# andyp223/ErasureCodedPIR

Measured on AMD Instinct MI355X. Metric: device-resident shard GiB/s per PIR query, 1/2/4/8 MI355X; bit-exact vs CPU, higher is better.
Workload: dtype u8; 1 GPU; north_star target shape: one shard 2^24 x 1 KiB, DPF depth 24, p=2; records=16777216, record_bytes=1024, parties=2, num_rounds=1, records_per_gpu=16777216, dpf_depth=24, parallelism=single, step=one PIR query: its own DPF key and tree, one full pass over the shard

## Files before the change

### erasurecodedpir_amd/csrc/pir_bits.h

```cpp
#pragma once
#include <stdint.h>

#if defined(__HIPCC__)
#include <hip/hip_runtime.h>
#define PIR_HD __host__ __device__ __forceinline__
#else
#define PIR_HD inline
#endif

namespace pir {

template <int S>
PIR_HD void bit_swap(uint32_t& a, uint32_t& b, uint32_t m) {
  const uint32_t t = ((a >> S) ^ b) & m;
  b ^= t;
  a ^= t << S;
}

PIR_HD void transpose8x32(uint32_t (&x)[8]) {
  bit_swap<4>(x[0], x[4], 0x0F0F0F0Fu); bit_swap<4>(x[1], x[5], 0x0F0F0F0Fu);
  bit_swap<4>(x[2], x[6], 0x0F0F0F0Fu); bit_swap<4>(x[3], x[7], 0x0F0F0F0Fu);
  bit_swap<2>(x[0], x[2], 0x33333333u); bit_swap<2>(x[1], x[3], 0x33333333u);
  bit_swap<2>(x[4], x[6], 0x33333333u); bit_swap<2>(x[5], x[7], 0x33333333u);
  bit_swap<1>(x[0], x[1], 0x55555555u); bit_swap<1>(x[2], x[3], 0x55555555u);
  bit_swap<1>(x[4], x[5], 0x55555555u); bit_swap<1>(x[6], x[7], 0x55555555u);
}

PIR_HD void transpose32(uint32_t (&a)[32]) {
#pragma unroll
  for (int k = 0; k < 16; ++k) bit_swap<16>(a[k], a[k + 16], 0x0000FFFFu);
#pragma unroll
  for (int k = 0; k < 32; ++k)
    if (!(k & 8)) bit_swap<8>(a[k], a[k + 8], 0x00FF00FFu);
#pragma unroll
  for (int k = 0; k < 32; ++k)
    if (!(k & 4)) bit_swap<4>(a[k], a[k + 4], 0x0F0F0F0Fu);
#pragma unroll
  for (int k = 0; k < 32; ++k)
    if (!(k & 2)) bit_swap<2>(a[k], a[k + 2], 0x33333333u);
#pragma unroll
  for (int k = 0; k < 32; ++k)
    if (!(k & 1)) bit_swap<1>(a[k], a[k + 1], 0x55555555u);
}

}
```

### erasurecodedpir_amd/csrc/pir_scan_t.hip

```cpp
#include "pir_bits.h"
#include <stdlib.h>
#include <type_traits>
#include "pir_kernels.h"

namespace pir {

constexpr int kScanTWaves = kScanTThreads / 64;

__device__ __forceinline__ uint32_t gf_xtime4_t(uint32_t x) {
  return ((x & 0x7f7f7f7fu) << 1) ^ (((x >> 7) & 0x01010101u) * 0x1du);
}

template <int NQ, int NRP>
__global__ __launch_bounds__(kScanTThreads) __attribute__((amdgpu_waves_per_eu(kScanTWavesPerEU)))
void k_scan_t(const uint8_t* __restrict__ shard, uint64_t nrec, uint32_t pitch, uint32_t cpr,
              const uint8_t* __restrict__ c, uint8_t* __restrict__ slabs, int accumulate,
              uint32_t ckey, uint64_t ckoff) {
  static_assert(NRP == 4 || NRP == 8, "coefficient words of 32 or 64 bits");
  static_assert(NQ >= 1 && NQ <= NRP, "rounds");
  constexpr int WD = NRP / 4;
  constexpr int GW = kColGroupLanes;
  __shared__ alignas(8) uint32_t tab[kScanTWaves][256 * WD];
  __shared__ uint32_t red[NQ * GW];
  __shared__ uint32_t next_chunk;
  for (int i = threadIdx.x; i < NQ * GW; i += blockDim.x) red[i] = 0;
  const bool dyn = (accumulate >> 1) & 1;
  accumulate &= 1;

  const uint32_t lane = threadIdx.x & 63;
  const uint32_t wv = __builtin_amdgcn_readfirstlane(threadIdx.x >> 6);
  const uint64_t wave = (uint64_t)blockIdx.x * kScanTWaves + wv;
  const uint64_t nwaves = (uint64_t)gridDim.x * kScanTWaves;
  const uint32_t chunk = blockIdx.y * kColGroupLanes + lane;
  const bool active = chunk < cpr;
  const uint64_t r0 = dyn ? (uint64_t)blockIdx.x * kScanTWaves * nrec / nwaves : wave * nrec / nwaves;
  const uint64_t r1 = dyn ? ((uint64_t)blockIdx.x + 1) * kScanTWaves * nrec / nwaves : (wave + 1) * nrec / nwaves;
  uint32_t* const tw = &tab[wv][0];
  if (dyn) {
    if (threadIdx.x == 0) next_chunk = 0;
    __syncthreads();
  }

  uint32_t Zt[32][WD];
#pragma unroll
  for (int j = 0; j < 32; ++j)
#pragma unroll
    for (int d = 0; d < WD; ++d) Zt[j][d] = 0;

  if (r1 > r0) {
    const uint32_t nrows = (uint32_t)(r1 - r0);
    const __amdgpu_buffer_rsrc_t rs = __builtin_amdgcn_make_buffer_rsrc(
        (void*)(shard + r0 * pitch), (short)0, (int)(nrows * pitch), kBufRsrcWord3);
    const uint32_t voff = (active ? chunk : 0u) * 4u;
    auto load_rel = [&](uint32_t rel) __attribute__((always_inline)) {
      return (uint32_t)__builtin_amdgcn_raw_buffer_load_b32(rs, voff, rel < nrows ? rel * pitch : 0u, 2);
    };
    auto coefs64 = [&](uint32_t rb) __attribute__((always_inline)) {
      const uint32_t rl = rb + lane;
      uint2 cw = make_uint2(0, 0);
      if (rl < nrows) {
        const uint64_t row = r0 + rl;
        if (ckey == 0) {
          const uint8_t* p = c + row * NRP;
          if constexpr (NRP == 8) cw = *reinterpret_cast<const uint2*>(p);
          else cw.x = *reinterpret_cast<const uint32_t*>(p);
        } else {
          uint64_t w = 0;
          for (uint32_t g = 0; g * ckey < (uint32_t)NRP; ++g) {
            const uint8_t* p = c + g * ckoff + row * ckey;
            const uint64_t v = ckey == 1 ? *p : (ckey == 2 ? *reinterpret_cast<const uint16_t*>(p)
                                                           : *reinterpret_cast<const uint32_t*>(p));
            w |= v << (8 * g * ckey);
          }
          cw = make_uint2((uint32_t)w, (uint32_t)(w >> 32));
        }
      }
      return cw;
    };
    uint32_t lm[6];
#pragma unroll
    for (int r = 0; r < 6; ++r) lm[r] = ((lane >> r) & 1u) ? 0xffffffffu : 0u;

    const uint32_t nch = (nrows + 63) / 64;
    auto claim = [&]() __attribute__((always_inline)) -> uint32_t {
      uint32_t v = 0;
      if (lane == 0)
        v = __hip_atomic_fetch_add(&next_chunk, 1u, __ATOMIC_RELAXED, __HIP_MEMORY_SCOPE_WORKGROUP);
      return (uint32_t)__builtin_amdgcn_readfirstlane(v);
    };
    uint32_t cur = dyn ? claim() : 0u;
    uint32_t nxt = dyn ? (cur < nch ? claim() : nch) : 1u;
    auto seq_row = [&](uint32_t k) __attribute__((always_inline)) -> uint32_t {
      return k < 64 ? cur * 64 + k : (nxt < nch ? nxt * 64 + (k - 64) : nrows);
    };
    uint32_t x[16];
#pragma unroll
    for (int u = 0; u < 16; ++u) x[u] = load_rel(seq_row((uint32_t)u));
    uint2 cw = cur < nch ? coefs64(cur * 64) : make_uint2(0, 0);
    for (; cur < nch;) {
      const uint32_t rb = cur * 64;
      const uint2 cwn = nxt < nch ? coefs64(nxt * 64) : make_uint2(0, 0);
      const uint32_t nb = nrows - rb < 64 ? nrows - rb : 64;
      for (uint32_t j0 = 0; j0 < nb; j0 += 16) {
#pragma unroll
        for (int g = 0; g < 2; ++g) {
          const uint32_t j = j0 + 8 * g;
#pragma unroll
          for (int d = 0; d < WD; ++d) {
            uint32_t w[8];
#pragma unroll
            for (int r = 0; r < 8; ++r)
              w[r] = (uint32_t)__builtin_amdgcn_readlane((int)(d ? cw.y : cw.x), (int)(j + r));
            uint32_t e = 0;
#pragma unroll
            for (int r = 0; r < 6; ++r) e = __builtin_amdgcn_bitop3_b32(e, w[r], lm[r], 0x78);
            const uint32_t e6 = e ^ w[6], e7 = e ^ w[7];
            tw[lane * WD + d] = e;
            tw[(lane + 64) * WD + d] = e6;
            tw[(lane + 128) * WD + d] = e7;
            tw[(lane + 192) * WD + d] = e6 ^ w[7];
          }
          __builtin_amdgcn_wave_barrier();
          uint32_t (&R)[8] = *reinterpret_cast<uint32_t(*)[8]>(&x[8 * g]);
          transpose8x32(R);
          uint32_t id[32];
#pragma unroll
          for (int jj = 0; jj < 32; ++jj) id[jj] = (R[jj & 7] >> (8 * (jj >> 3))) & 0xffu;
          using Ent = typename std::conditional<WD == 2, uint2, uint32_t>::type;
          const Ent* te = reinterpret_cast<const Ent*>(tw);
          Ent ta[8], tb[8];
          auto issue = [&](Ent (&t)[8], int ch) __attribute__((always_inline)) {
#pragma unroll
            for (int q = 0; q < 8; ++q) t[q] = te[id[8 * ch + q]];
            __builtin_amdgcn_sched_barrier(0);
          };
          auto fold = [&](const Ent (&t)[8], int ch) __attribute__((always_inline)) {
#pragma unroll
            for (int q = 0; q < 8; ++q) {
              if constexpr (WD == 2) {
                Zt[8 * ch + q][0] ^= t[q].x;
                Zt[8 * ch + q][1] ^= t[q].y;
              } else {
                Zt[8 * ch + q][0] ^= t[q];
              }
            }
            __builtin_amdgcn_sched_barrier(0);
          };
          issue(ta, 0);
          issue(tb, 1);
          fold(ta, 0);
          issue(ta, 2);
          fold(tb, 1);
          issue(tb, 3);
          fold(ta, 2);
          fold(tb, 3);
          __builtin_amdgcn_wave_barrier();
#pragma unroll
          for (int r = 0; r < 8; ++r) x[8 * g + r] = load_rel(seq_row(j + 16 + r));
          __builtin_amdgcn_sched_barrier(0);
        }
      }
      cw = cwn;
      cur = nxt;
      nxt = dyn ? (cur < nch ? claim() : nch) : cur + 1;
    }
  }
  __syncthreads();
  if (active) {
#pragma unroll
    for (int d = 0; d < WD; ++d) {
      if (4 * d >= NQ) continue;
      uint32_t Y[32];
#pragma unroll
      for (int j = 0; j < 32; ++j) Y[j] = Zt[j][d];
      transpose32(Y);
#pragma unroll
      for (int a4 = 0; a4 < 4; ++a4) {
        const int a = 4 * d + a4;
        if (a >= NQ) continue;
        uint32_t acc = Y[8 * a4 + 7];
#pragma unroll
        for (int b = 6; b >= 0; --b) acc = gf_xtime4_t(acc) ^ Y[8 * a4 + b];
        if (acc) atomicXor(&red[a * GW + lane], acc);
      }
    }
  }
  __syncthreads();
  uint32_t* slab = reinterpret_cast<uint32_t*>(slabs) +
                   ((uint64_t)blockIdx.y * gridDim.x + blockIdx.x) * (NQ * GW);
  if (accumulate)
    for (int i = threadIdx.x; i < NQ * GW; i += blockDim.x) slab[i] ^= red[i];
  else
    for (int i = threadIdx.x; i < NQ * GW; i += blockDim.x) slab[i] = red[i];
}

static int scan_t_mode() {
  const char* v = getenv("PIR_SCAN_T");
  return v ? atoi(v) : 1;
}
bool scan_t_enabled() { return scan_t_mode() != 0; }

bool scan_t_shape(int nq, int nrp, uint32_t pitch, bool prefer) {
  if (!scan_t_enabled() || nq < 4 || nq > 8 || nq > nrp || (nrp != 4 && nrp != 8)) return false;
  if (pitch % 4 != 0 || pitch / 4 < (uint32_t)kColGroupLanes) return false;
  return nq >= 6 || pitch / 8 < (uint32_t)kColGroupLanes || prefer || scan_t_mode() == 2;
}

template <int NQ, int NRP>
static hipError_t scan_t_launch(const ScanShape& sh, const uint8_t* d_shard, uint64_t nrec,
                                const uint8_t* d_c, uint8_t* d_slabs, int acc, hipStream_t s) {
  if (sh.ckey != 0 && (sh.ckey > 4 || NRP % sh.ckey != 0)) return hipErrorInvalidValue;
  hipLaunchKernelGGL((k_scan_t<NQ, NRP>), sh.grid, dim3(kScanTThreads), 0, s, d_shard, nrec,
                     sh.pitch, sh.cpr, d_c, d_slabs, acc, sh.ckey, sh.ckoff);
  return hipGetLastError();
}

hipError_t launch_scan_t(const ScanShape& sh, const uint8_t* d_shard, uint64_t nrec,
                         const uint8_t* d_c, uint8_t* d_slabs, int acc, hipStream_t s) {
  if (sh.threads != kScanTThreads || sh.vec != 1 || !sh.uniform) return hipErrorInvalidValue;
#define PIR_ST(NQ, NRP) \
  if (sh.nq == NQ && sh.nrp == NRP) return scan_t_launch<NQ, NRP>(sh, d_shard, nrec, d_c, d_slabs, acc, s)
  PIR_ST(4, 4); PIR_ST(4, 8); PIR_ST(5, 8); PIR_ST(6, 8); PIR_ST(7, 8); PIR_ST(8, 8);
#undef PIR_ST
  return hipErrorInvalidValue;
}

}
```

Before: 11590 GiB/s.

## Switch scan lookup tables from 8-bit to 4-bit subset-XOR tables

Builds 16-entry subset-XOR tables (4 rows each) once per 64-row chunk using DPP broadcasts, instead of rebuilding 256-entry 8-row tables with readlane for every 8-row group. Indices become nibbles taken from a cheaper 4x32 bit transpose. Each fold combines two table reads with a three-input XOR (bitop3). This cuts table construction and transpose ALU work and shrinks LDS use, but doubles the number of LDS lookups per row group.

New measurement: 11900 GiB/s, median of 6. 2.7% higher.

```diff
diff --git a/erasurecodedpir_amd/csrc/pir_bits.h b/erasurecodedpir_amd/csrc/pir_bits.h
--- a/erasurecodedpir_amd/csrc/pir_bits.h
+++ b/erasurecodedpir_amd/csrc/pir_bits.h
@@ -15,6 +15,11 @@
   const uint32_t t = ((a >> S) ^ b) & m;
   b ^= t;
   a ^= t << S;
+}
+
+PIR_HD void transpose4x32(uint32_t (&x)[4]) {
+  bit_swap<2>(x[0], x[2], 0x33333333u); bit_swap<2>(x[1], x[3], 0x33333333u);
+  bit_swap<1>(x[0], x[1], 0x55555555u); bit_swap<1>(x[2], x[3], 0x55555555u);
 }
 
 PIR_HD void transpose8x32(uint32_t (&x)[8]) {
diff --git a/erasurecodedpir_amd/csrc/pir_scan_t.hip b/erasurecodedpir_amd/csrc/pir_scan_t.hip
--- a/erasurecodedpir_amd/csrc/pir_scan_t.hip
+++ b/erasurecodedpir_amd/csrc/pir_scan_t.hip
@@ -20,7 +20,10 @@
   static_assert(NQ >= 1 && NQ <= NRP, "rounds");
   constexpr int WD = NRP / 4;
   constexpr int GW = kColGroupLanes;
-  __shared__ alignas(8) uint32_t tab[kScanTWaves][256 * WD];
+  using Ent = typename std::conditional<WD == 2, uint2, uint32_t>::type;
+  constexpr int ESH = WD == 2 ? 3 : 2;
+  constexpr int kTabBytes = 16 << ESH;
+  __shared__ alignas(128) uint32_t tab[kScanTWaves][16 * kTabBytes / 4];
   __shared__ uint32_t red[NQ * GW];
   __shared__ uint32_t next_chunk;
   for (int i = threadIdx.x; i < NQ * GW; i += blockDim.x) red[i] = 0;
@@ -77,9 +80,31 @@
       }
       return cw;
     };
-    uint32_t lm[6];
-#pragma unroll
-    for (int r = 0; r < 6; ++r) lm[r] = ((lane >> r) & 1u) ? 0xffffffffu : 0u;
+    const uint32_t q2 = (lane & 1u) ? 0xffffffffu : 0u, q3 = (lane & 2u) ? 0xffffffffu : 0u;
+    auto build_tables = [&](const uint2& cw) __attribute__((always_inline)) {
+      uint32_t e[4][WD];
+#pragma unroll
+      for (int d = 0; d < WD; ++d) {
+        const int s = (int)(d ? cw.y : cw.x);
+        const uint32_t w0 = (uint32_t)__builtin_amdgcn_update_dpp(0, s, 0x00, 0xf, 0xf, false);
+        const uint32_t w1 = (uint32_t)__builtin_amdgcn_update_dpp(0, s, 0x55, 0xf, 0xf, false);
+        const uint32_t w2 = (uint32_t)__builtin_amdgcn_update_dpp(0, s, 0xaa, 0xf, 0xf, false);
+        const uint32_t w3 = (uint32_t)__builtin_amdgcn_update_dpp(0, s, 0xff, 0xf, 0xf, false);
+        e[0][d] = (w2 & q2) ^ (w3 & q3);
+        e[1][d] = e[0][d] ^ w0;
+        e[2][d] = e[0][d] ^ w1;
+        e[3][d] = e[1][d] ^ w1;
+      }
+      __builtin_amdgcn_wave_barrier();
+      uint4* const dst = reinterpret_cast<uint4*>(tw) + lane * WD;
+      if constexpr (WD == 2) {
+        dst[0] = make_uint4(e[0][0], e[0][1], e[1][0], e[1][1]);
+        dst[1] = make_uint4(e[2][0], e[2][1], e[3][0], e[3][1]);
+      } else {
+        dst[0] = make_uint4(e[0][0], e[1][0], e[2][0], e[3][0]);
+      }
+      __builtin_amdgcn_wave_barrier();
+    };
 
     const uint32_t nch = (nrows + 63) / 64;
     auto claim = [&]() __attribute__((always_inline)) -> uint32_t {
@@ -101,47 +126,40 @@
       const uint32_t rb = cur * 64;
       const uint2 cwn = nxt < nch ? coefs64(nxt * 64) : make_uint2(0, 0);
       const uint32_t nb = nrows - rb < 64 ? nrows - rb : 64;
+      build_tables(cw);
       for (uint32_t j0 = 0; j0 < nb; j0 += 16) {
+        const char* const tj = reinterpret_cast<const char*>(tw) + j0 / 4 * kTabBytes;
 #pragma unroll
         for (int g = 0; g < 2; ++g) {
           const uint32_t j = j0 + 8 * g;
-#pragma unroll
-          for (int d = 0; d < WD; ++d) {
-            uint32_t w[8];
-#pragma unroll
-            for (int r = 0; r < 8; ++r)
-              w[r] = (uint32_t)__builtin_amdgcn_readlane((int)(d ? cw.y : cw.x), (int)(j + r));
-            uint32_t e = 0;
-#pragma unroll
-            for (int r = 0; r < 6; ++r) e = __builtin_amdgcn_bitop3_b32(e, w[r], lm[r], 0x78);
-            const uint32_t e6 = e ^ w[6], e7 = e ^ w[7];
-            tw[lane * WD + d] = e;
-            tw[(lane + 64) * WD + d] = e6;
-            tw[(lane + 128) * WD + d] = e7;
-            tw[(lane + 192) * WD + d] = e6 ^ w[7];
-          }
-          __builtin_amdgcn_wave_barrier();
-          uint32_t (&R)[8] = *reinterpret_cast<uint32_t(*)[8]>(&x[8 * g]);
-          transpose8x32(R);
-          uint32_t id[32];
-#pragma unroll
-          for (int jj = 0; jj < 32; ++jj) id[jj] = (R[jj & 7] >> (8 * (jj >> 3))) & 0xffu;
-          using Ent = typename std::conditional<WD == 2, uint2, uint32_t>::type;
-          const Ent* te = reinterpret_cast<const Ent*>(tw);
+          uint32_t (&L)[4] = *reinterpret_cast<uint32_t(*)[4]>(&x[8 * g]);
+          uint32_t (&H)[4] = *reinterpret_cast<uint32_t(*)[4]>(&x[8 * g + 4]);
+          transpose4x32(L);
+          transpose4x32(H);
+          const char* const tg = tj + g * (2 * kTabBytes);
           Ent ta[8], tb[8];
-          auto issue = [&](Ent (&t)[8], int ch) __attribute__((always_inline)) {
-#pragma unroll
-            for (int q = 0; q < 8; ++q) t[q] = te[id[8 * ch + q]];
+          auto issue = [&](Ent (&t)[8], int s) __attribute__((always_inline)) {
+            uint32_t lo = (s & 1) ? L[s >> 1] >> (4 - ESH) : L[s >> 1] << ESH;
+            uint32_t hi = (s & 1) ? H[s >> 1] >> (4 - ESH) : H[s >> 1] << ESH;
+            lo &= 0x0f0f0f0fu << ESH;
+            hi &= 0x0f0f0f0fu << ESH;
+            asm volatile("" : "+v"(lo), "+v"(hi));
+#pragma unroll
+            for (int b = 0; b < 4; ++b) {
+              t[2 * b] = *reinterpret_cast<const Ent*>(tg + ((lo >> (8 * b)) & 0xffu));
+              t[2 * b + 1] = *reinterpret_cast<const Ent*>(tg + kTabBytes + ((hi >> (8 * b)) & 0xffu));
+            }
             __builtin_amdgcn_sched_barrier(0);
           };
-          auto fold = [&](const Ent (&t)[8], int ch) __attribute__((always_inline)) {
-#pragma unroll
-            for (int q = 0; q < 8; ++q) {
+          auto fold = [&](const Ent (&t)[8], int s) __attribute__((always_inline)) {
+#pragma unroll
+            for (int b = 0; b < 4; ++b) {
+              uint32_t (&z)[WD] = Zt[8 * b + 4 * (s & 1) + (s >> 1)];
               if constexpr (WD == 2) {
-                Zt[8 * ch + q][0] ^= t[q].x;
-                Zt[8 * ch + q][1] ^= t[q].y;
+                z[0] = __builtin_amdgcn_bitop3_b32(z[0], t[2 * b].x, t[2 * b + 1].x, 0x96);
+                z[1] = __builtin_amdgcn_bitop3_b32(z[1], t[2 * b].y, t[2 * b + 1].y, 0x96);
               } else {
-                Zt[8 * ch + q][0] ^= t[q];
+                z[0] = __builtin_amdgcn_bitop3_b32(z[0], t[2 * b], t[2 * b + 1], 0x96);
               }
             }
             __builtin_amdgcn_sched_barrier(0);
@@ -153,8 +171,15 @@
           fold(tb, 1);
           issue(tb, 3);
           fold(ta, 2);
+          issue(ta, 4);
           fold(tb, 3);
-          __builtin_amdgcn_wave_barrier();
+          issue(tb, 5);
+          fold(ta, 4);
+          issue(ta, 6);
+          fold(tb, 5);
+          issue(tb, 7);
+          fold(ta, 6);
+          fold(tb, 7);
 #pragma unroll
           for (int r = 0; r < 8; ++r) x[8 * g + r] = load_rel(seq_row(j + 16 + r));
           __builtin_amdgcn_sched_barrier(0);
```
